# hihixuyang/LQR-Obstacles

Hardware: AMD Instinct MI355X
Metric: agent-pair LQR-obstacle evals/sec (higher is better)
Workload: dtype f64

## Files before the change

lqr-obstacles_amd/csrc/lqro_plan.hpp:

```cpp
#pragma once

#include <algorithm>
#include <climits>
#include <cstddef>
#include <cstdlib>
#include <vector>

namespace lqro {

struct StepKnobs {
  int hot_on;
  int hot_split;
  int hot_spec;
  long hot_max_inside;
  double hot_t, hot_r;
  int qside;
  int qside_pct;
  int qspare;
  int qbalance;
  int qhull_inline;
  int qhull_big;
  int qhull_flags;
  int hull_big_only;
  int local_hull;
  int lhull_prof;
  int side_cus;
  int lside_cus;
  int early_lp;
};

inline int env_int(const char* name, int dflt) {
  const char* e = std::getenv(name);
  return e ? std::atoi(e) : dflt;
}
inline long env_long(const char* name, long dflt) {
  const char* e = std::getenv(name);
  return e ? std::atol(e) : dflt;
}
inline double env_double(const char* name, double dflt) {
  const char* e = std::getenv(name);
  return e ? std::atof(e) : dflt;
}

inline StepKnobs knobs_from_env(int n_cu) {
  StepKnobs k{};
  k.qhull_big = env_int("LQRO_QHULL_BIG", 0) != 0;
  k.side_cus = std::max(0, std::min(n_cu / 2, env_int("LQRO_SIDE_HULL_CUS", (3 * n_cu) / 8)));
  k.hull_big_only = env_int("LQRO_HULL_BIG", 0) != 0;
  k.local_hull = env_int("LQRO_LOCAL_HULL", 1) != 0;
  k.lside_cus = std::max(0, std::min(n_cu / 2, env_int("LQRO_LOCAL_SIDE_CUS", (3 * n_cu) / 16)));
  k.hot_on = env_int("LQRO_HOT", 1) != 0;
  k.hot_t = env_double("LQRO_HOT_T", 3.0);
  k.hot_r = env_double("LQRO_HOT_R", 3.0);
  k.lhull_prof = env_int("LQRO_LHULL_PROFILE", 0) != 0;
  k.hot_max_inside = env_long("LQRO_HOT_MAX_INSIDE", -1L);
  k.early_lp = env_int("LQRO_EARLY_LP", 1) != 0;
  k.hot_split = env_int("LQRO_HOT_SPLIT", 1) != 0;
  k.hot_spec = env_int("LQRO_HOT_SPEC", 1) != 0;
  k.qspare = env_int("LQRO_QHULL_SPARE", 4);
  k.qside_pct = std::max(1, std::min(100, env_int("LQRO_QHULL_SIDE_PCT", 100)));
  k.qside = env_int("LQRO_QSIDE", 0) != 0;
  k.qhull_inline = env_int("LQRO_QHULL_INLINE_BIG", 1) != 0;
  k.qhull_flags = env_int("LQRO_QHULL_FLAGS", 23);
  k.qbalance = env_int("LQRO_QHULL_BALANCE", 1) != 0;
  return k;
}

struct StepFeedback {
  unsigned long long inside;
  unsigned long long sweep_work;
  unsigned long long build_work;
  unsigned long long build_max;
  unsigned long long retried;
  unsigned long long unused[3];
};
static_assert(sizeof(StepFeedback) == 8 * sizeof(unsigned long long), "one slot is 8 words");
constexpr StepFeedback kNoFeedback = {~0ull, 0ull, 0ull, 0ull, 0ull, {0ull, 0ull, 0ull}};

struct StepShape {
  int n_cu, nrows;
  int npr;
  int nbr_k;
  size_t hnp;
  int per_agent, qhull_order;
  int phase;
  bool has_newv;
  bool newv_is_callers;
  int waves, lds_wave, wave_doubles;
  size_t hull_lds_max_hnp;
  size_t hull_lds_doubles;
  int hull_cwaves;
  size_t qhull_lds_doubles;
  size_t lp_lds_max;
  int early_lp_max_npr;
  int row_big;
  int extra_planes = 0;
  int n_obs = 0;
};

struct StepPlan {
  int npr;
  long slots;
  bool lds_ok;
  int side_waves;
  int qside_waves;
  bool hot;
  int side;
  int nwait;
  bool split, spec, qside;
  bool early, early_internal;
  int row_split;
  unsigned nblk, nside;
  int big_inline, row_lp, row_target;
};

inline int qhull_side_balance(int n, double w_sweep, double w_build, double b_max) {
  const int kmax = n - n / 8;
  double best = 1e300;
  std::vector<double> t((size_t)kmax + 1, 0.0);
  for (int k = 1; k <= kmax; ++k) {
    t[k] = std::max(std::max(b_max, 1.15 * w_build / k), w_sweep / (double)(n - k));
    best = std::min(best, t[k]);
  }
  for (int k = kmax; k >= 1; --k)
    if (t[k] <= 1.02 * best) return k;
  return kmax;
}

inline StepPlan plan_step(const StepShape& S, const StepKnobs& K, const StepFeedback& F, bool known) {
  StepPlan p{};
  const int cols = S.npr + S.n_obs;
  const int npr = S.nbr_k > 0 ? std::min(S.nbr_k, cols) : cols;
  p.npr = npr;
  const bool lds_ok = S.hnp <= S.hull_lds_max_hnp && !K.hull_big_only;
  const long slots = (long)S.nrows * npr;
  const long side_room = (long)S.hull_lds_doubles - S.lds_wave;
  const int side_waves = side_room > 0 ? (int)std::min<long>(std::min(S.hull_cwaves, S.waves),
                                                              side_room / S.wave_doubles) : 0;
  const unsigned long long inside_prev = F.inside;
  const double w_sweep = 1e-5 * (double)F.sweep_work;
  const double w_build = 1e-5 * (double)F.build_work;
  const double b_max = 1e-5 * (double)F.build_max;
  const unsigned long long retried_prev = F.retried;
  const bool lhull = K.local_hull || S.qhull_order;
  int side = lhull ? K.lside_cus : K.side_cus;
  const unsigned long long qspare =
      !known ? 0ull : K.qspare >= 0 ? (unsigned long long)K.qspare : inside_prev / 16 + 4;
  unsigned long long qwant =
      known ? (inside_prev * (unsigned long long)K.qside_pct + 99ull) / 100ull + qspare : 0ull;
  if (S.qhull_order && K.qbalance && known && w_sweep > 0.0 && b_max > 0.0)
    qwant = std::min(qwant, (unsigned long long)qhull_side_balance(S.n_cu, w_sweep, w_build, b_max));
  if (S.qhull_order) {
    const unsigned long long want = known ? qwant : (unsigned long long)(S.n_cu / 2);
    side = (int)std::min<unsigned long long>((unsigned long long)(S.n_cu - S.n_cu / 8),
                                             std::max<unsigned long long>((unsigned long long)side, want));
  } else if (lhull) {
    if (known)
      side = (int)std::max<unsigned long long>(
          (unsigned long long)side,
          std::min<unsigned long long>(S.n_cu / 2, (inside_prev * 10ull + 36ull) / 37ull));
  } else if (known && inside_prev > 2ull * (unsigned long long)side) {
    side = std::min(S.n_cu / 2, (4 * side) / 3);
  }
  const long max_inside = K.hot_max_inside >= 0 ? K.hot_max_inside
                          : S.qhull_order     ? LONG_MAX
                          : (lhull ? 16L * std::max(side, S.n_cu / 2) : 4L * side);
  const bool crowded = known && inside_prev > (unsigned long long)max_inside;
  const bool hot = K.hot_on && S.n_cu >= 64 && slots >= 65536 && S.nbr_k <= 0 && !crowded && side >= 1 &&
                   (known || !S.qhull_order) &&
                   (lhull || (lds_ok && S.hnp <= 16383 && side_waves >= 1));
  const int nwait = hot ? side : 0;
  p.row_split = std::max(1, std::min(16, (2 * S.n_cu + S.nrows - 1) / S.nrows));
  const long qside_room = (long)S.qhull_lds_doubles - S.lds_wave;
  const int qside_waves = qside_room > 0 ? (int)std::min<long>(3, qside_room / S.wave_doubles) : 0;
  const bool qside = hot && K.qside && S.qhull_order && !K.qhull_big && qside_waves >= 1;
  if (qside && !S.per_agent) p.row_split = std::max(p.row_split, std::min(16, std::max(1, npr / 128)));
  const bool early = hot && K.early_lp && S.qhull_order && !K.qhull_big && S.phase != 2 && S.nbr_k <= 0 &&
                     ((size_t)npr + (size_t)S.extra_planes) * 32 <= S.lp_lds_max && S.has_newv;
  p.early = early;
  p.early_internal = early && !S.newv_is_callers;
  const int units = S.nrows * p.row_split;
  const unsigned nblk = (unsigned)std::min(units, S.n_cu - nwait);
  const unsigned nside = (unsigned)std::max(0, std::min(units - (int)nblk, nwait));
  const bool split = hot && S.qhull_order && K.hot_split && !qside && !K.qhull_big && known &&
                     qwant <= (unsigned long long)nwait;
  const bool spec = split && K.hot_spec;
  p.slots = slots; p.lds_ok = lds_ok; p.side_waves = side_waves; p.qside_waves = qside_waves;
  p.hot = hot; p.side = side; p.nwait = nwait;
  p.split = split; p.spec = spec; p.qside = qside;
  p.nblk = nblk; p.nside = nside;
  p.big_inline = K.qhull_inline && !K.qhull_big && (S.hnp > 10000 || retried_prev > 0) ? 1 : 0;
  p.row_lp = npr <= S.early_lp_max_npr && S.extra_planes <= 0 ? 1 : 0;
  p.row_target = p.row_split * S.row_big;
  return p;
}

}
```

lqr-obstacles_amd/csrc/lqro_qhull3.hpp:

```cpp
#pragma once
#include "lqro_qhull.hpp"
#include "lqro_qhull3_prof.hpp"
#include "lqro_lp.hpp"

namespace lqro {

#ifndef Q3_NEWCAP
#define Q3_NEWCAP 128
#endif
#ifndef Q3_VISCAP
#define Q3_VISCAP 192
#endif
#define Q3_MOVCAP 16
#define Q3_HZCAP 24
#define Q3_COPCAP 8
#define Q3_FSTK 512
#define Q3_ND (Q3_NEWCAP + Q3_MOVCAP)
#define Q3_WAVES 4
#define Q3_HR 4
#ifndef Q3_W0_SLEEP
#define Q3_W0_SLEEP 1
#endif
#ifndef Q3_W1_SLEEP
#define Q3_W1_SLEEP 1
// ... 418 lines not shown
  int cur[3] = {q3_nb(W, L, startfacet, 0), q3_nb(W, L, startfacet, 1), q3_nb(W, L, startfacet, 2)};
  for (;;) {
    double q[3][4];
    int fl[3], nn[3][3];
    for (int k = 0; k < 3; k++) q3_get(W, L, cur[k], q[k], nn[k], &fl[k]);
    bool seen3[3] = {false, false, false};
    for (int t = 0; t < nvis; t++) {
      const int v = q3_col<G>(vis[64 * t]);
      seen3[0] |= v == cur[0]; seen3[1] |= v == cur[1]; seen3[2] |= v == cur[2];
    }
    for (int k = 0; k < 3; k++) {
      const int nb = cur[k];
      const bool seen = seen3[k] || (k >= 1 && nb == cur[0]) || (k == 2 && nb == cur[1]);
      if (seen) continue;
      if (nvis == Q3_HZCAP) { lstatus |= QHS_CAPACITY | Q3_CAPBIT(QHS_CAP_HZ); return bestfacet; }
      q3_col_st<G>(vis[64 * nvis], (unsigned short)nb);
      nvis++;
      if (!(fl[k] & QF_FLIPPED)) {
        const double dist = q3_distq(q[k], p);
        if (dist > *bestdist) {
          minsearch = dist - searchdist;
          if (dist > *bestdist + searchdist) ncop = 0;
          bestfacet = nb;
          *bestdist = dist;
        } else if (dist < minsearch) {
          continue;
        }
      }
      if (nextfacet >= 0) {
        if (ncop == Q3_COPCAP) { lstatus |= QHS_CAPACITY | Q3_CAPBIT(QHS_CAP_COP); return bestfacet; }
        q3_col_st<G>(cop[64 * ncop++], nextfacet);
      }
      nextfacet = nb;
      nextnb[0] = nn[k][0]; nextnb[1] = nn[k][1]; nextnb[2] = nn[k][2];
    }
    if (nextfacet >= 0) {
      nextfacet = -1;
      cur[0] = nextnb[0]; cur[1] = nextnb[1]; cur[2] = nextnb[2];
      continue;
    }
    if (!ncop) break;
    int facet;
    if (ncop == 1) { facet = q3_col<G>(cop[0]); ncop = 0; }
    else facet = q3_col<G>(cop[64 * --ncop]);
    cur[0] = q3_nb(W, L, facet, 0); cur[1] = q3_nb(W, L, facet, 1); cur[2] = q3_nb(W, L, facet, 2);
  }
  return bestfacet;
}

template <bool G>
__device__ inline int q3_findbestnew(const Q3W& W, const Q3S& S, const Q3L& L, const double* p, int s0,
                                     double* dist, int bestoutside, int* isoutside, int& lstatus, const Q3Col& C) {
  double bestdist = -DBL_MAX / 2;
  int bestfacet = -1;
  const double distoutside = fmax(2 * S.MINoutside, S.max_outside);
  *isoutside = 1;
  const int total = S.nnew + S.nmov;
  auto fetch = [&](int t, int& f, int& fl, double* q) {
    if (t < S.nnew - s0 || t >= S.nnew - s0 + S.nmov) {
      const int u = t < S.nnew - s0 ? s0 + t : t - (S.nnew - s0) - S.nmov;
      f = L.nslot[u];
      const double4 v = q3_lds(*reinterpret_cast<const double4*>(L.npl + 4 * u));
      q[0] = v.x; q[1] = v.y; q[2] = v.z; q[3] = v.w;
      fl = L.nflag[u];
    } else {
      f = L.movf[t - (S.nnew - s0)];
      q3_pl(W, L, f, q);
      fl = q3_fa(W, L, f);
    }
  };
  for (int t0 = 0; t0 < total; t0 += 4) {
    int f[4], fl[4];
    double q[4][4];
#pragma unroll
    for (int k = 0; k < 4; k++) {
      f[k] = -1; fl[k] = QF_FLIPPED;
      if (t0 + k < total) fetch(t0 + k, f[k], fl[k], q[k]);
    }
#pragma unroll
    for (int k = 0; k < 4; k++) {
      if (fl[k] & QF_FLIPPED) continue;
      const double d = q3_distq(q[k], p);
      if (d > bestdist) {
        bestfacet = f[k];
        if (!bestoutside && d >= distoutside) { *dist = d; return bestfacet; }
        bestdist = d;
      }
    }
  }
  bestfacet = q3_findbesthorizon<G>(W, S, L, p, bestfacet >= 0 ? bestfacet : L.nslot[s0], &bestdist, lstatus, C);
  *dist = bestdist;
  if (bestdist < S.MINoutside) *isoutside = 0;
  return bestfacet;
}

__device__ inline int q3_sharpnewfacets(const Q3S& S, const Q3L& L, int lane) {
  if (S.nnew == 0) return 0;
  const bool q0 = L.npl[0] > 0, q1 = L.npl[1] > 0, q2 = L.npl[2] > 0;
  bool diff = false;
  for (int t = lane; t < S.nnew; t += 64) {
    const double* n = L.npl + 4 * t;
    diff |= (n[0] > 0) != q0 || (n[1] > 0) != q1 || (n[2] > 0) != q2;
  }
  return __ballot(diff) != 0ull;
}

template <bool G>
__device__ inline int q3_locate(const Q3W& W, const Q3S& S, const Q3L& L, const double* p, int s0, int sharp,
                                double* bestdist_out, int* isoutside, int* trigger, int& lstatus, const Q3Col& C) {
  *trigger = 0;
  if (sharp == 2) return q3_findbestnew<G>(W, S, L, p, s0, bestdist_out, 1, isoutside, lstatus, C);
  if (S.findbestnew) return q3_findbestnew<G>(W, S, L, p, s0, bestdist_out, 0, isoutside, lstatus, C);
  double bestdist = -DBL_MAX / 2;
  int bestu = -1;
  *isoutside = 1;
  unsigned long long m0 = 0ull, m1 = 0ull;
  if (!(L.nflag[s0] & QF_FLIPPED)) {
    const double d = q3_distq(L.npl + 4 * s0, p);
    if (d >= S.MINoutside) { *bestdist_out = d; return L.nslot[s0]; }
    bestdist = d;
    bestu = s0;
  }
  if (s0 < 64) m0 |= 1ull << s0; else m1 |= 1ull << (s0 - 64);
  int u = s0;
  while (u >= 0) {
    int nxt = -1;
    const int cand[2] = {L.nn1[u], L.nn2[u]};
    const int cfl[2] = {L.nflag[cand[0]], L.nflag[cand[1]]};
    double cq[2][4];
#pragma unroll
    for (int k = 0; k < 2; k++) {
      const double4 v = q3_lds(*reinterpret_cast<const double4*>(L.npl + 4 * cand[k]));
      cq[k][0] = v.x; cq[k][1] = v.y; cq[k][2] = v.z; cq[k][3] = v.w;
    }
#pragma unroll
    for (int k = 0; k < 2; k++) {
      const int c = cand[k];
      const bool was = c < 64 ? (m0 >> c) & 1ull : (m1 >> (c - 64)) & 1ull;
      if (was) continue;
      if (c < 64) m0 |= 1ull << c; else m1 |= 1ull << (c - 64);
      if (!(cfl[k] & QF_FLIPPED)) {
        const double d = q3_distq(cq[k], p);
        if (d > bestdist) {
          if (d >= S.MINoutside) { *bestdist_out = d; return L.nslot[c]; }
          bestu = c;
          bestdist = d;
          nxt = c;
          break;
        }
      }
    }
    u = nxt;
  }
  if (bestu < 0) return q3_findbestnew<G>(W, S, L, p, 0, bestdist_out, 0, isoutside, lstatus, C);
  if (!S.notsharp && bestdist < -S.DISTround) {
    *trigger = 1;
    if (sharp) return q3_findbestnew<G>(W, S, L, p, bestu, bestdist_out, 0, isoutside, lstatus, C);
  }
  const int bf = q3_findbesthorizon<G>(W, S, L, p, L.nslot[bestu], &bestdist, lstatus, C);
  *bestdist_out = bestdist;
  if (bestdist < S.MINoutside) *isoutside = 0;
  return bf;
}

__device__ __forceinline__ bool q3_in_movf(const Q3S& S, const Q3L& L, int f) {
  for (int t = 0; t < S.nmov; t++)
    if (L.movf[t] == f) return true;
  return false;
}

__device__ __forceinline__ HullPt q3_seqpt(const Q3W& W, const Q3L& L, int nvis, bool init, int pos, int* start) {
  HullPt r;
  if (init) {
    const int q = W.pq[pos];
    r.x = W.Pr[3 * (size_t)q]; r.y = W.Pr[3 * (size_t)q + 1]; r.z = W.Pr[3 * (size_t)q + 2];
    r.q = q;
    r.pad = 0;
    *start = 0;
    return r;
  }
  int a = 0, b = nvis - 1;
  while (a < b) {
    const int mid = (a + b) >> 1;
    if (L.vinc[mid] > pos) b = mid;
    else a = mid + 1;
  }
  *start = L.repl[a] >= 0 ? L.repl[a] : 0;
  const int q = W.sb[L.vsoff[a] + pos - (L.vinc[a] - L.vscnt[a])];
  r.x = W.Pr[3 * (size_t)q]; r.y = W.Pr[3 * (size_t)q + 1]; r.z = W.Pr[3 * (size_t)q + 2];
  r.q = q;
  r.pad = 0;
  return r;
}

__device__ __forceinline__ int q3_ld_acq(const int* p) {
  return __hip_atomic_load(p, __ATOMIC_ACQUIRE, __HIP_MEMORY_SCOPE_WORKGROUP);
}
__device__ __forceinline__ void q3_st_rel(int* p, int v) {
  __hip_atomic_store(p, v, __ATOMIC_RELEASE, __HIP_MEMORY_SCOPE_WORKGROUP);
}
__device__ __forceinline__ void q3_st_rel_lds(int* p, int v) {
  __builtin_amdgcn_fence(__ATOMIC_RELEASE, "workgroup", "local");
  __hip_atomic_store(p, v, __ATOMIC_RELAXED, __HIP_MEMORY_SCOPE_WORKGROUP);
}
__device__ __forceinline__ int q3_wait(const int* p, int v, bool ne) {
  int x = q3_ld_acq(p);
  for (long w = 0; (ne ? x == v : x != v) && w < (1l << 24); ++w) {
    __builtin_amdgcn_s_sleep(Q3_W0_SLEEP);
    x = q3_ld_acq(p);
  }
  return x;
}

template <bool G>
__device__ __forceinline__ void q3_chunk_locate(const Q3W& W, const Q3S& S, const Q3L& L, int c, int from, int np,
                                                int sharp, bool init, int lane, const HullPt& pre, int prestart,
                                                int prec, HullPt& pt, int& f, double& d, int& isout, int& trig,
                                                int& ls, const Q3Col& C) {
  const int pos = c + lane;
  pt = pre;
  f = -1; d = 0.0; isout = 0; trig = 0;
  if (pos >= from && pos < np) {
    int start = prestart;
    if (c != prec) pt = q3_seqpt(W, L, S.nvis, init, pos, &start);
    const double p[3] = {pt.x, pt.y, pt.z};
    f = q3_locate<G>(W, S, L, p, start, sharp, &d, &isout, &trig, ls, C);
  }
}

__device__ inline bool q3_help(const Q3W& W, Q3L& L, int lane, const Q3Col& C) {
  const unsigned v = (unsigned)q3_ld_acq(reinterpret_cast<const int*>(&L.hctl));
  if (v == 0u) return false;
  const int k = (int)(v & 0xffffu);
  if (k >= L.hq_end || k >= hl_ld(&L.hcons) + Q3_HR) return false;
  int got = 0;
  if (lane == 0) {
    __hip_atomic_fetch_add(&L.hbusy, 1, __ATOMIC_SEQ_CST, __HIP_MEMORY_SCOPE_WORKGROUP);
    unsigned e = v;
    got = __hip_atomic_compare_exchange_strong(&L.hctl, &e, v + 1u, __ATOMIC_SEQ_CST, __ATOMIC_SEQ_CST,
                                               __HIP_MEMORY_SCOPE_WORKGROUP);
    if (!got) __hip_atomic_fetch_add(&L.hbusy, -1, __ATOMIC_SEQ_CST, __HIP_MEMORY_SCOPE_WORKGROUP);
  }
  if (!__builtin_amdgcn_readfirstlane(got)) return false;
#ifdef LQRO_QHULL_LONGPROF
  const unsigned long long th0 = __builtin_amdgcn_s_memrealtime();
#endif
  Q3S S;
  S.MINvisible = L.c_dist[0]; S.MAXcoplanar = L.c_dist[1]; S.DISTround = L.c_dist[2];
  S.MINoutside = 2 * S.MINvisible;
  S.findbestnew = L.hq_findbestnew; S.notsharp = L.hq_notsharp;
  S.nnew = L.hq_nnew; S.nmov = L.hq_nmov; S.nvis = L.hq_nvis;
  S.max_outside = L.hq_max_outside;
  HullPt pt, pre;
  pre.x = pre.y = pre.z = 0.0; pre.q = -1; pre.pad = 0;
  int f, isout, trig, ls = 0;
  double d;
  const int from = L.hq_from, np = L.hq_np, pos = 64 * k + lane;
  q3_chunk_locate<true>(W, S, L, 64 * k, from, np, L.hq_sharp, L.hq_init != 0, lane, pre, 0, -1, pt, f, d, isout,
                        trig, ls, C);
#ifdef LQRO_QHULL_LONGPROF
  const unsigned long long th1 = __builtin_amdgcn_s_memrealtime();
#endif
  int kind = 0, dst = -1, dfa = 0;
  if (pos >= from && pos < np) {
    if (isout) {
      dst = f;
      dfa = q3_fa(W, L, f);
      if (!(dfa & QF_NEW) && (q3_cc(W, L, f) & 0xffffu) == 0 && !q3_in_movf(S, L, f)) kind |= 4;
    } else if (d >= -S.MAXcoplanar && d > S.max_outside) {
      kind |= 2;
    }
    if (trig) kind |= 1;
  }
  const bool old = dst >= 0 && !(dfa & QF_NEW);
  const int b = k % Q3_HR;
  L.hr_d[64 * b + lane] = d;
  L.hr_f[64 * b + lane] = (unsigned short)dst;
  L.hr_k[64 * b + lane] = (unsigned short)(kind | (old ? 8 : 0) | ((dst >= 0 && !old ? (dfa >> 8) + 1 : 0) << 8));
  const int st = qh_wave_or(ls);
  if (lane == 0) {
    L.hr_ls[b] = st;
    q3_st_rel_lds(&L.hr_st[b], k + 1);
    __hip_atomic_fetch_add(&L.hbusy, -1, __ATOMIC_SEQ_CST, __HIP_MEMORY_SCOPE_WORKGROUP);
#ifdef LQRO_QHULL_LONGPROF
    const unsigned long long th2 = __builtin_amdgcn_s_memrealtime();
    atomicAdd(&L.hprof[0], 1ull);
    atomicAdd(&L.hprof[1], th1 - th0);
    atomicAdd(&L.hprof[2], th2 - th0);
#endif
  }
  return true;
}

__device__ inline void q3_locate_seq(const Q3W& W, Q3S& S, Q3L& L, int np, int sharp, bool init, int lane,
                                     const HullPt& pre, int prestart, bool havepre, int& rg, double& rd,
                                     HullPt& rpt) {
  for (int t = lane; t < Q3_NEWCAP; t += 64) L.pcnt[t] = 0;
  S.nold = 0;
  rg = -1;
  rd = 0.0;
  rpt = pre;
  hl_sync();
  const bool help = np > 64 && (L.qflags & 1);
  const Q3Col C0 = q3_col0(L, lane);
  auto post = [&](int from2) {
    S.hgen = S.hgen % 32767 + 1;
    if (lane == 0) {
      L.hq_end = (np + 63) >> 6; L.hq_from = from2; L.hq_np = np; L.hq_sharp = sharp; L.hq_init = init ? 1 : 0;
      L.hq_findbestnew = S.findbestnew; L.hq_notsharp = S.notsharp; L.hq_nnew = S.nnew; L.hq_nmov = S.nmov;
      L.hq_nvis = S.nvis; L.hq_max_outside = S.max_outside;
      L.hcons = from2 >> 6;
      for (int b = 0; b < Q3_HR; b++) L.hr_st[b] = 0;
      q3_st_rel(reinterpret_cast<int*>(&L.hctl), (int)(((unsigned)S.hgen << 16) | (unsigned)((from2 >> 6) + 1)));
    }
  };
  auto stop = [&]() {
    if (lane == 0) __hip_atomic_exchange(&L.hctl, 0u, __ATOMIC_SEQ_CST, __HIP_MEMORY_SCOPE_WORKGROUP);
    int b = __hip_atomic_load(&L.hbusy, __ATOMIC_SEQ_CST, __HIP_MEMORY_SCOPE_WORKGROUP);
    for (long w = 0; b != 0 && w < (1l << 24); ++w) {
      __builtin_amdgcn_s_sleep(Q3_W0_SLEEP);
      b = __hip_atomic_load(&L.hbusy, __ATOMIC_SEQ_CST, __HIP_MEMORY_SCOPE_WORKGROUP);
    }
    if (b != 0) S.status |= QHS_CAPACITY | QHS_TIMEOUT;
  };
  int from = 0;
  while (from < np && !(S.status & QHS_CAPACITY)) {
    int ev_pos = np, ev_kind = 0, ev_dst = -1;
    double ev_d = 0.0;
    if (help) post(from);
    bool first = help;
    for (int c = from & ~63; c < np; c += 64) {
      Q3C(23, 1);
      const int pos = c + lane;
      const bool act = pos >= from && pos < np;
      int kind = 0, ls = 0, dst = -1, dfa = 0;
      double d = 0.0;
      HullPt pt = pre;
      int f = -1, isout = 0, trig = 0;
      bool mine = !help || first;
      if (help && !first) {
        const int k = c >> 6, b = k % Q3_HR;
        int st = q3_ld_acq(&L.hr_st[b]);
        if (st != k + 1) {
          int m = 0;
          if (lane == 0) {
            unsigned e = __hip_atomic_load(&L.hctl, __ATOMIC_RELAXED, __HIP_MEMORY_SCOPE_WORKGROUP);
            if ((e & 0xffffu) == (unsigned)k)
              m = __hip_atomic_compare_exchange_strong(&L.hctl, &e, e + 1u, __ATOMIC_RELAXED, __ATOMIC_RELAXED,
                                                       __HIP_MEMORY_SCOPE_WORKGROUP);
          }
          mine = __builtin_amdgcn_readfirstlane(m) != 0;
#ifdef LQRO_QHULL_LONGPROF
          const unsigned long long tw0 = __builtin_amdgcn_s_memrealtime();
#endif
          if (!mine) st = q3_wait(&L.hr_st[b], k + 1, false);
#ifdef LQRO_QHULL_LONGPROF
          if (!mine) S.pf.lp_hwait += __builtin_amdgcn_s_memrealtime() - tw0;
#endif
        }
#ifdef LQRO_QHULL_LONGPROF
        if (mine) S.pf.lp_own++; else S.pf.lp_got++;
#endif
        int kv = 0;
        if (!mine) {
          if (st != k + 1) { S.status |= QHS_CAPACITY | QHS_TIMEOUT; break; }
          const int fv = L.hr_f[64 * b + lane];
          kv = L.hr_k[64 * b + lane];
          ls = L.hr_ls[b];
          dst = fv == 0xffff ? -1 : fv;
          kind = act ? kv & 7 : 0;
          dfa = (kv & 8) ? 0 : (((kv >> 8) - 1) << 8) | QF_NEW;
          d = L.hr_d[64 * b + lane];
        }
      }
      first = false;
      Q3T(12);
      if (mine) q3_chunk_locate<false>(W, S, L, c, from, np, sharp, init, lane, pre, prestart, havepre ? 0 : -1, pt, f,
                                       d, isout, trig, ls, C0);
      Q3T(13);
      if (mine && act) {
        if (isout) {
          dst = f;
          dfa = q3_fa(W, L, f);
          if (!(dfa & QF_NEW) && (q3_cc(W, L, f) & 0xffffu) == 0 && !q3_in_movf(S, L, f)) kind |= 4;
        } else if (d >= -S.MAXcoplanar && d > S.max_outside) {
          kind |= 2;
        }
        if (trig) kind |= 1;
      }
      S.status |= qh_wave_or(ls);
      if (help && lane == 0) q3_st_rel_lds(&L.hcons, (c >> 6) + 1);
      const unsigned long long b = __ballot(kind != 0);
      const int last = b ? __ffsll((long long)b) - 1 : 63;
      const bool fin = act && lane <= last;
      int g = -1;
      if (fin && dst >= 0 && (dfa & QF_NEW)) {
        g = dfa >> 8;
        atomicAdd(&L.pcnt[g], 1);
      }
      unsigned long long old = __ballot(fin && dst >= 0 && !(dfa & QF_NEW));
      while (old) {
        const int l = __ffsll((long long)old) - 1;
        old &= old - 1;
        const int f = __builtin_amdgcn_readlane(dst, l);
        int k = -1;
        for (int t = 0; t < S.nold; t++)
          if (L.oldf[t] == f) k = t;
        if (k < 0) {
          if (S.nold == Q3_MOVCAP) { S.status |= QHS_CAPACITY | Q3_CAPBIT(QHS_CAP_MOV); continue; }
          k = S.nold++;
          if (lane == 0) { L.oldf[k] = f; L.pcnt[Q3_NEWCAP + k] = 0; L.dfac[Q3_NEWCAP + k] = f; }
          hl_sync();
        }
        if (lane == 0) L.pcnt[Q3_NEWCAP + k]++;
        if (lane == l) g = Q3_NEWCAP + k;
        hl_sync();
      }
      if (fin) {
        rg = g;
        rd = d;
        rpt = pt;
        if (np > 64) {
          W.pdst[pos] = g;
          W.pdd[pos] = d;
        }
      }
      hl_sync();
      Q3T(14);
      if (b) {
        ev_pos = c + last;
        ev_kind = __builtin_amdgcn_readlane(kind, last);
        ev_dst = __builtin_amdgcn_readlane(dst, last);
        ev_d = hl_rl(d, last);
        break;
      }
    }
#ifdef LQRO_QHULL_LONGPROF
    const unsigned long long ts0 = __builtin_amdgcn_s_memrealtime();
#endif
    if (help) stop();
#ifdef LQRO_QHULL_LONGPROF
    if (help) {
      S.pf.lp_stop += __builtin_amdgcn_s_memrealtime() - ts0;
      S.pf.lp_posts++;
      if (ev_pos < np) S.pf.lp_ev++;
    }
#endif
    if (S.status & QHS_CAPACITY) return;
    if (ev_pos < np) {
      Q3C(24, 1);
      if (ev_kind & 1) {
        if (sharp) S.findbestnew = 1;
        else S.notsharp = 1;
      }
      if (ev_kind & 2) S.max_outside = ev_d;
      if (ev_kind & 4) {
        const int f = ev_dst;
        if (S.nmov == Q3_MOVCAP) {
          S.status |= QHS_CAPACITY | Q3_CAPBIT(QHS_CAP_MOV);
          return;
        }
        if (lane == 0) {
          L.movf[S.nmov] = f;
          if (init) {
            int t0 = 0;
            for (int t = 0; t < S.nnew; t++)
              if (L.nslot[t] == f) t0 = t;
            for (int t = t0; t + 1 < S.nnew; t++) {
              L.nslot[t] = L.nslot[t + 1];
              for (int k = 0; k < 4; k++) L.npl[4 * t + k] = L.npl[4 * (t + 1) + k];
              L.nflag[t] = L.nflag[t + 1];
            }
            double q[4];
            q3_pl(W, L, f, q);
            L.nslot[S.nnew - 1] = f;
            for (int k = 0; k < 4; k++) L.npl[4 * (S.nnew - 1) + k] = q[k];
            L.nflag[S.nnew - 1] = q3_fa(W, L, f);
          }
        }
        q3_set_key(W, L, f, S.keyc);
        S.keyc++;
        S.nmov++;
      }
      hl_sync();
    }
    from = ev_pos + 1;
  }
}

__device__ inline void q3_emit_bucket(const Q3W& W, Q3L& L, int lane, int b) {
  const int np = L.ej_np, nd = L.ej_nd, ndnew = L.ej_ndnew, nvis = L.ej_nvis;
  const bool init = L.ej_init != 0;
  const int gl = lane < ndnew ? lane : Q3_NEWCAP + (lane - ndnew);
  const bool has = lane < nd && (lane & 3) == b && L.pcnt[gl];
  int Rc = 0, Rch = -1, Ro = 0;
  double Rm = 0.0, Rx = 0.0, Ry = 0.0, Rz = 0.0;
  if (has) {
    Rc = L.dcnt[gl]; Rm = L.dmax[gl]; Rch = L.dchamp[gl]; Ro = L.doff[gl];
    Rx = L.dchp[3 * gl]; Ry = L.dchp[3 * gl + 1]; Rz = L.dchp[3 * gl + 2];
  }
  const unsigned long long ltmask = (1ull << lane) - 1ull;
  int ng = -1;
  double ndd = 0.0;
  HullPt npt;
  npt.x = npt.y = npt.z = 0.0; npt.q = -1; npt.pad = 0;
  auto ldc = [&](int c) {
    const int pos = c + lane;
    ng = -1;
    ndd = 0.0;
    if (pos < np) {
      ng = W.pdst[pos];
      ndd = W.pdd[pos];
      int st;
      npt = q3_seqpt(W, L, nvis, init, pos, &st);
    }
  };
  ldc(0);
  for (int c = 0; c < np; c += 64) {
    const int g = ng;
    const double dd = ndd;
    const HullPt pt = npt;
    if (c + 64 < np) ldc(c + 64);
    const int i = g < 0 ? -1 : (g < Q3_NEWCAP ? g : ndnew + (g - Q3_NEWCAP));
    const bool mine = i >= 0 && (i & 3) == b;
    unsigned long long todo = __ballot(mine);
    int wpos = -1, wr = 0;
    while (todo) {
      const int lead = __ffsll((long long)todo) - 1;
      const int gg = __builtin_amdgcn_readlane(g, lead);
      const unsigned long long grp = __ballot(mine && g == gg);
      todo &= ~grp;
      const int l = __builtin_amdgcn_readlane(i, lead);
      int cnt = __builtin_amdgcn_readlane(Rc, l), champ = __builtin_amdgcn_readlane(Rch, l);
      double mx = hl_rl(Rm, l), cx = hl_rl(Rx, l), cy = hl_rl(Ry, l), cz = hl_rl(Rz, l);
      q3_place(grp, lane, ltmask, dd, pt, __builtin_amdgcn_readlane(Ro, l), W.SB, cnt, mx, champ, cx, cy, cz, wpos,
               wr);
      if (lane == l) { Rc = cnt; Rm = mx; Rch = champ; Rx = cx; Ry = cy; Rz = cz; }
    }
    if (wpos >= 0) W.sb[wpos] = wr;
  }
  if (has) {
    L.dcnt[gl] = Rc; L.dmax[gl] = Rm; L.dchamp[gl] = Rch;
    L.dchp[3 * gl] = Rx; L.dchp[3 * gl + 1] = Ry; L.dchp[3 * gl + 2] = Rz;
  }
}

__device__ __forceinline__ int q3_emit_claim(Q3L& L, int lane) {
  int k = -1;
  if (lane == 0) {
    for (;;) {
      unsigned v = (unsigned)q3_ld_acq(reinterpret_cast<const int*>(&L.ectl));
      if (v == 0u || (v & 0xffu) >= 4u) break;
      unsigned e = v;
      if (__hip_atomic_compare_exchange_strong(&L.ectl, &e, v + 1u, __ATOMIC_ACQ_REL, __ATOMIC_RELAXED,
                                               __HIP_MEMORY_SCOPE_WORKGROUP)) {
        k = (int)(v & 0xffu);
        break;
      }
    }
  }
  return __builtin_amdgcn_readfirstlane(k);
}

__device__ inline bool q3_emit_help(const Q3W& W, Q3L& L, int lane) {
  const unsigned v = (unsigned)q3_ld_acq(reinterpret_cast<const int*>(&L.ectl));
  if (v == 0u || (v & 0xffu) >= 4u) return false;
  const int k = q3_emit_claim(L, lane);
  if (k < 0) return false;
  q3_emit_bucket(W, L, lane, k);
  if (lane == 0) {
    __builtin_amdgcn_fence(__ATOMIC_RELEASE, "workgroup");
    __hip_atomic_fetch_add(&L.edone, 1, __ATOMIC_RELEASE, __HIP_MEMORY_SCOPE_WORKGROUP);
  }
  return true;
}

__device__ inline void q3_emit_seq(const Q3W& W, Q3S& S, Q3L& L, int np, int ndnew, bool init, int lane, int rg,
                                   double rd, const HullPt& rpt) {
  if (S.status & QHS_CAPACITY) return;
  if (!init && np <= 64 && S.nold == 0 && ndnew <= 64) {
    const int g = lane;
    int pc = 0, f = 0;
    if (g < ndnew) { f = L.nslot[g]; pc = L.pcnt[g]; }
    const int inc = q3_scan_add(pc);
    const int top = S.sbtop + __builtin_amdgcn_readlane(inc, 63);
    if (top > W.SB) {
      S.status |= QHS_CAPACITY | Q3_CAPBIT(QHS_CAP_SB);
      return;
    }
    const int doff = S.sbtop + inc - pc;
    S.sbtop = top;
    Q3T(15);
    int dcnt = 0, dchamp = -1;
    double dmax = 0.0, dx = 0.0, dy = 0.0, dz = 0.0;
    const unsigned long long ltmask = (1ull << lane) - 1ull;
    const int rgl = lane < np ? rg : -1;
    unsigned long long todo = __ballot(rgl >= 0);
    int wpos = -1, wr = 0;
    Q3T(16);
    while (todo) {
      const int lead = __ffsll((long long)todo) - 1;
      const int gg = __builtin_amdgcn_readlane(rgl, lead);
      const unsigned long long grp = __ballot(rgl == gg);
      todo &= ~grp;
      int cnt = 0, champ = -1;
      double mx = 0.0, cx = 0.0, cy = 0.0, cz = 0.0;
      q3_place(grp, lane, ltmask, rd, rpt, __builtin_amdgcn_readlane(doff, gg), W.SB, cnt, mx, champ, cx, cy, cz,
               wpos, wr);
      Q3C(25, 1);
      if (lane == gg) { dcnt = cnt; dmax = mx; dchamp = champ; dx = cx; dy = cy; dz = cz; }
    }
    if (wpos >= 0) W.sb[wpos] = wr;
    Q3T(17);
    if (g < ndnew && pc) {
      W.sb[doff + dcnt - 1] = dchamp;
      W.soff[f] = doff;
      W.fdist[f] = dmax;
      q3_set_cc(W, L, f, (unsigned)dcnt | ((unsigned)dchamp << 16));
    }
    const bool has = g < ndnew && pc > 0;
    const unsigned long long b = __ballot(has);
    int qt = S.qtail;
    if (has) {
      const int at = qt + __popcll(b & ltmask);
      if (at < W.QC) {
        W.fq[at] = f;
        W.fqk[at] = S.key0_last + (unsigned)g;
        HullPt r;
        r.x = dx; r.y = dy; r.z = dz; r.q = dchamp; r.pad = 0;
        W.fqc[at] = r;
      }
    }
    qt += __popcll(b);
    if (qt > W.QC) S.status |= QHS_CAPACITY | Q3_CAPBIT(QHS_CAP_FACETS);
    S.qtail = qt;
    hl_sync();
    Q3T(18);
    return;
  }
  const int nd = ndnew + S.nold;
  int base = S.sbtop;
  for (int c0 = 0; c0 < nd; c0 += 64) {
    const int i = c0 + lane;
    int size = 0, g = -1, cnt0 = 0;
    if (i < nd) {
      g = i < ndnew ? i : Q3_NEWCAP + (i - ndnew);
      if (g < Q3_NEWCAP) L.dfac[g] = L.nslot[g];
      if (L.pcnt[g]) {
        cnt0 = g < Q3_NEWCAP ? 0 : (int)(q3_cc(W, L, L.dfac[g]) & 0xffffu);
        size = cnt0 + L.pcnt[g];
      }
    }
    const int inc = q3_scan_add(size);
    if (size) {
      L.doff[g] = base + inc - size;
      L.dcnt[g] = cnt0;
      L.dmax[g] = 0.0;
      L.dchamp[g] = -1;
    }
    base += __builtin_amdgcn_readlane(inc, 63);
  }
  if (base > W.SB) {
    S.status |= QHS_CAPACITY | Q3_CAPBIT(QHS_CAP_SB);
    return;
  }
  S.sbtop = base;
  hl_sync();
  for (int k = 0; k < S.nold; k++) {
    const int g = Q3_NEWCAP + k;
    const int f = L.dfac[g];
    const int cnt0 = L.dcnt[g];
    if (!L.pcnt[g] || !cnt0) continue;
    const int off0 = W.soff[f];
    const int off = L.doff[g];
    for (int t = lane; t < cnt0 - 1; t += 64) W.sb[off + t] = W.sb[off0 + t];
    const int chq = W.sb[off0 + cnt0 - 1];
    const double fd = W.fdist[f];
    if (lane == 0) {
      L.dchamp[g] = chq;
      L.dchp[3 * g] = W.Pr[3 * (size_t)chq]; L.dchp[3 * g + 1] = W.Pr[3 * (size_t)chq + 1];
      L.dchp[3 * g + 2] = W.Pr[3 * (size_t)chq + 2];
      L.dmax[g] = fd;
    }
    hl_sync();
  }
  hl_sync();
  Q3T(15);
  if (np > 64 && nd <= 64 && (L.qflags & 16)) {
    S.egen = S.egen % 0xffffff + 1;
    if (lane == 0) {
      L.ej_np = np; L.ej_nd = nd; L.ej_ndnew = ndnew; L.ej_init = init ? 1 : 0; L.ej_nvis = S.nvis;
      L.edone = 0;
      q3_st_rel(reinterpret_cast<int*>(&L.ectl), (int)((unsigned)S.egen << 8));
    }
    int mine = 0;
    for (int k = q3_emit_claim(L, lane); k >= 0; k = q3_emit_claim(L, lane)) {
      q3_emit_bucket(W, L, lane, k);
      ++mine;
    }
    hl_sync();
    int dn = q3_ld_acq(&L.edone);
    for (long w = 0; dn != 4 - mine && w < (1l << 24); ++w) {
      __builtin_amdgcn_s_sleep(Q3_W0_SLEEP);
      dn = q3_ld_acq(&L.edone);
    }
    if (lane == 0) __hip_atomic_store(&L.ectl, 0u, __ATOMIC_RELAXED, __HIP_MEMORY_SCOPE_WORKGROUP);
    if (dn != 4 - mine) { S.status |= QHS_CAPACITY | QHS_TIMEOUT; return; }
  } else {
  const bool inl = nd <= 64 && (L.qflags & 2);
  int Rc = 0, Rch = -1, Ro = 0;
  double Rm = 0.0, Rx = 0.0, Ry = 0.0, Rz = 0.0;
  if (inl && lane < nd) {
    const int g = lane < ndnew ? lane : Q3_NEWCAP + (lane - ndnew);
    if (L.pcnt[g]) {
      Rc = L.dcnt[g]; Rm = L.dmax[g]; Rch = L.dchamp[g]; Ro = L.doff[g];
      Rx = L.dchp[3 * g]; Ry = L.dchp[3 * g + 1]; Rz = L.dchp[3 * g + 2];
    }
  }
  int ng = -1;
  double ndd = 0.0;
  HullPt npt = rpt;
  auto ldc = [&](int c) {
    const int pos = c + lane;
    ng = -1;
    ndd = 0.0;
    if (pos < np) {
      ng = W.pdst[pos];
      ndd = W.pdd[pos];
      int st;
      npt = q3_seqpt(W, L, S.nvis, init, pos, &st);
    }
  };
  if (np > 64) ldc(0);
  for (int c = 0; c < np; c += 64) {
    const int pos = c + lane;
    const bool act = pos < np;
    int g = rg;
    double dd = rd;
// ... 1734 lines not shown
```

Before: 59.05 million.

## Let qhull partition helpers run ahead speculatively in findbestnew mode

Enables new qhull flag bits (32, 64) by default. Bit 32 marks non-sharp non-init partition passes as notsharp up front. Bit 64 posts helper work with findbestnew already set, so helper waves keep locating points past a sharp trigger event instead of stopping and re-posting. The main wave then continues from the event without a new post, and it either owns chunks or waits on a held chunk's status. The aim is to remove stop and re-post round trips in the cooperative point-partition loop, at the cost of more complex synchronisation and a possible change in which facet each point is assigned to.

```diff
diff --git a/lqr-obstacles_amd/csrc/lqro_plan.hpp b/lqr-obstacles_amd/csrc/lqro_plan.hpp
--- a/lqr-obstacles_amd/csrc/lqro_plan.hpp
+++ b/lqr-obstacles_amd/csrc/lqro_plan.hpp
@@ -61,7 +61,7 @@
   k.qside_pct = std::max(1, std::min(100, env_int("LQRO_QHULL_SIDE_PCT", 100)));
   k.qside = env_int("LQRO_QSIDE", 0) != 0;
   k.qhull_inline = env_int("LQRO_QHULL_INLINE_BIG", 1) != 0;
-  k.qhull_flags = env_int("LQRO_QHULL_FLAGS", 23);
+  k.qhull_flags = env_int("LQRO_QHULL_FLAGS", 119);
   k.qbalance = env_int("LQRO_QHULL_BALANCE", 1) != 0;
   return k;
 }
diff --git a/lqr-obstacles_amd/csrc/lqro_qhull3.hpp b/lqr-obstacles_amd/csrc/lqro_qhull3.hpp
--- a/lqr-obstacles_amd/csrc/lqro_qhull3.hpp
+++ b/lqr-obstacles_amd/csrc/lqro_qhull3.hpp
@@ -744,12 +744,16 @@
   rpt = pre;
   hl_sync();
   const bool help = np > 64 && (L.qflags & 1);
+  if (sharp == 0 && !init && (L.qflags & 32)) S.notsharp = 1;
+  const bool a2 = help && sharp == 1 && (L.qflags & 64);
+  bool ahead = false;
   const Q3Col C0 = q3_col0(L, lane);
   auto post = [&](int from2) {
     S.hgen = S.hgen % 32767 + 1;
+    ahead = a2 && !S.findbestnew;
     if (lane == 0) {
       L.hq_end = (np + 63) >> 6; L.hq_from = from2; L.hq_np = np; L.hq_sharp = sharp; L.hq_init = init ? 1 : 0;
-      L.hq_findbestnew = S.findbestnew; L.hq_notsharp = S.notsharp; L.hq_nnew = S.nnew; L.hq_nmov = S.nmov;
+      L.hq_findbestnew = ahead ? 1 : S.findbestnew; L.hq_notsharp = S.notsharp; L.hq_nnew = S.nnew; L.hq_nmov = S.nmov;
       L.hq_nvis = S.nvis; L.hq_max_outside = S.max_outside;
       L.hcons = from2 >> 6;
       for (int b = 0; b < Q3_HR; b++) L.hr_st[b] = 0;
@@ -766,11 +770,13 @@
     if (b != 0) S.status |= QHS_CAPACITY | QHS_TIMEOUT;
   };
   int from = 0;
+  bool posted = false;
   while (from < np && !(S.status & QHS_CAPACITY)) {
     int ev_pos = np, ev_kind = 0, ev_dst = -1;
     double ev_d = 0.0;
-    if (help) post(from);
-    bool first = help;
+    if (help && !posted) post(from);
+    bool first = help && (!posted || (from & 63) != 0);
+    posted = false;
     for (int c = from & ~63; c < np; c += 64) {
       Q3C(23, 1);
       const int pos = c + lane;
@@ -780,10 +786,14 @@
       HullPt pt = pre;
       int f = -1, isout = 0, trig = 0;
       bool mine = !help || first;
+      const bool own = ahead && !S.findbestnew;
+      int held = -1;
       if (help && !first) {
         const int k = c >> 6, b = k % Q3_HR;
         int st = q3_ld_acq(&L.hr_st[b]);
-        if (st != k + 1) {
+        if (own && st == k + 1) {
+          mine = true;
+        } else if (st != k + 1) {
           int m = 0;
           if (lane == 0) {
             unsigned e = __hip_atomic_load(&L.hctl, __ATOMIC_RELAXED, __HIP_MEMORY_SCOPE_WORKGROUP);
@@ -795,6 +805,7 @@
 #ifdef LQRO_QHULL_LONGPROF
           const unsigned long long tw0 = __builtin_amdgcn_s_memrealtime();
 #endif
+          if (!mine && own) { mine = true; held = b; }
           if (!mine) st = q3_wait(&L.hr_st[b], k + 1, false);
 #ifdef LQRO_QHULL_LONGPROF
           if (!mine) S.pf.lp_hwait += __builtin_amdgcn_s_memrealtime() - tw0;
@@ -831,6 +842,10 @@
         if (trig) kind |= 1;
       }
       S.status |= qh_wave_or(ls);
+      if (held >= 0 && q3_wait(&L.hr_st[held], (c >> 6) + 1, false) != (c >> 6) + 1) {
+        S.status |= QHS_CAPACITY | QHS_TIMEOUT;
+        break;
+      }
       if (help && lane == 0) q3_st_rel_lds(&L.hcons, (c >> 6) + 1);
       const unsigned long long b = __ballot(kind != 0);
       const int last = b ? __ffsll((long long)b) - 1 : 63;
@@ -876,6 +891,13 @@
         ev_d = hl_rl(d, last);
         break;
       }
+    }
+    if (ahead && !S.findbestnew && ev_kind == 1 && ev_pos + 1 < np) {
+      Q3C(24, 1);
+      S.findbestnew = 1;
+      from = ev_pos + 1;
+      posted = true;
+      continue;
     }
 #ifdef LQRO_QHULL_LONGPROF
     const unsigned long long ts0 = __builtin_amdgcn_s_memrealtime();
```

Measured after the change: 59.81 million, median of 6. 1.3% higher.
